# stecrotti/MPSKit.jl

Hardware: AMD Instinct MI355X
Metric: DMRG sweeps/sec + ddAC matvec achieved-TFLOP/s, Heisenberg L=100 D=1024 fp64 (higher is better)
Workload: dtype f64; 1 GPU; Heisenberg S=1/2 FiniteMPS L=100 D=1024 d=2 W=5 fp64, 1-site DMRG sweep (2L-2 site updates), fixed Krylov budget 8 matvecs/site; parallelism=single GPU

## Files before the change

mpskit.jl_amd/csrc/mpsk_api.hip:

```cpp
#include <hip/hip_runtime.h>
#include <cstdio>
#include <cstdlib>
#include <cstring>
#include <cmath>
#include <algorithm>
#include <map>
#include <string>
#include <vector>
#include "mpsk.h"
#include "mpsk_internal.h"

using namespace mpsk;

static thread_local std::string g_err;
static int fail(int code, const std::string& msg) { g_err = msg; return code; }
#define HIPCHK(expr)                                                                        \
  do {                                                                                      \
    hipError_t e_ = (expr);                                                                 \
    if (e_ != hipSuccess)                                                                   \
      return fail(MPSK_ERR_HIP, std::string(#expr) + ": " + hipGetErrorString(e_));         \
  } while (0)
#define REQUIRE(cond, msg)                                                  \
  do {                                                                      \
    if (!(cond)) return fail(MPSK_ERR_INVALID, std::string(__func__) + ": " + (msg)); \
// ... 1074 lines not shown
  for (int q = 0; q < nblk; ++q) { g1.segA[q] = (int64_t)q * kb * Dlo; g1.segB[q] = (int64_t)q * kb * d * Dr; }
  g1.tag = 1;
  HIPCHK(gemm_f64(g1, c->stream));
  GemmArgs g3 = mk(T1, h->GRc, (double*)y, Dlo, Dr, Dr, (int64_t)Dlo * d, Dr, (int64_t)Dlo * d);
  g3.batch = d; g3.bsA = 0; g3.bsB = 0; g3.bsC = (int64_t)Dlo;
  g3.nseg = ns; g3.zsegA = h->zseg; g3.zsegB = h->zseg + (size_t)d * ns;
  g3.tabs_even = (Dlo % 2 == 0) && (Dr % 2 == 0);
  g3.tag = 1;
  HIPCHK(gemm_f64(g3, c->stream));
  return MPSK_OK;
}

int mpsk_hac_eigsolve_fixed(mpsk_hac* h, const void* x0, int m, void* const* V, void* scal, void* y, void* first_image) {
  REQUIRE(h && x0 && V && scal && y, "NULL argument");
  REQUIRE(m >= 1 && m <= 32, "needs 1 <= m <= 32");
  REQUIRE(h->mode != 2, "mpsk_hac_eigsolve_fixed: MPSK_F64 operators only");
  mpsk_ctx* c = h->ctx;
  HIPCHK(hipSetDevice(c->device));
  const int64_t n = (int64_t)h->Dlo * h->H->d * h->Dr;
  REQUIRE(h->Dlo == h->Dl, "mpsk_hac_eigsolve_fixed: the operator must be square (unsharded)");
  double* slot = (double*)scal;
  const int stride = 2 * m + 1;
  double* rbuf = slot + (size_t)m * stride;
  if (int rc = mpsk_vnormalize_dev(c, n, x0, V[0], nullptr)) return rc;
  for (int k = 0; k < m; ++k) {
    if (int rc = mpsk_hac_apply(h, V[k], 1, V[k + 1])) return rc;
    if (k == 0 && first_image) HIPCHK(hipMemcpyAsync(first_image, V[1], sizeof(double) * n, hipMemcpyDeviceToDevice, c->stream));
    HIPCHK(vec_cgs2((const double* const*)V, k + 1, (double*)V[k + 1], n, slot + (size_t)k * stride, c->d_partial, c->stream));
    HIPCHK(vec_scal_rsqrt_dev(slot + (size_t)k * stride + 2 * (k + 1), (double*)V[k + 1], n, c->stream));
  }
  HIPCHK(vec_ritz_small(slot, m, stride, rbuf, rbuf + 32, c->stream));
  HIPCHK(hipMemsetAsync(V[m + 1], 0, sizeof(double) * n, c->stream));
  HIPCHK(vec_multiaxpy((const double* const*)V, rbuf, m, 1.0, (double*)V[m + 1], n, c->stream));
  return mpsk_vnormalize_dev(c, n, V[m + 1], y, nullptr);
}

int mpsk_dC(mpsk_ctx* c, int W, int Dlo, int Dl, int Dr, const void* GL, const void* GR, const void* cm, void* y) {
  REQUIRE(c && GL && GR && cm && y, "NULL argument");
  REQUIRE(W > 0 && Dlo > 0 && Dl > 0 && Dr > 0, "dimensions must be positive");
  if (c->dtype == MPSK_C128)
    return dC_c128(c, W, Dlo, Dl, Dr, (const double*)GL, (const double*)GR, (const double*)cm, (double*)y);
  HIPCHK(hipSetDevice(c->device));
  const size_t slab = (size_t)Dlo * Dr;
  if (int rc = ensure_ws(c, sizeof(double) * slab * W)) return rc;
  double* T1 = (double*)c->ws;
  GemmArgs g1 = mk((const double*)GL, (const double*)cm, T1, Dlo, Dr, Dl, Dlo, Dl, Dlo);
  g1.batch = W; g1.bsA = (int64_t)Dlo * Dl; g1.bsB = 0; g1.bsC = (int64_t)slab;
  g1.tag = 1;
  HIPCHK(gemm_f64(g1, c->stream));
  std::vector<int64_t> sa, sb;
  for (int w = 0; w < W; ++w) { sa.push_back((int64_t)w * slab); sb.push_back((int64_t)w * Dr * Dr); }
  GemmArgs g3 = mk(T1, (const double*)GR, (double*)y, Dlo, Dr, Dr, Dlo, Dr, Dlo);
  g3.tag = 1;
  HIPCHK(gemm_segments(g3, sa, sb, c->stream));
  return MPSK_OK;
}

// ... 1398 lines not shown
  REQUIRE(n > 0, "bad n");
  REQUIRE(((uintptr_t)x % 16 == 0) && ((uintptr_t)y % 16 == 0), "operands must be 16-byte aligned");
  HIPCHK(hipSetDevice(c->device));
  HIPCHK(vec_diff_nrm2((const double*)x, (const double*)y, c->dtype == MPSK_C128 ? 2 * n : n, c->d_scal, c->d_partial,
                       c->stream));
  return fetch_scalars(c, 2, host_out);
}

int mpsk_vgs_step(mpsk_ctx* c, int64_t n, int k, const void* const* xs, void* y, double* host_out) {
  REQUIRE(c && xs && y && host_out, "NULL argument");
  REQUIRE(k > 0 && k <= MAXK && n > 0, "bad k or n");
  HIPCHK(hipSetDevice(c->device));
  HIPCHK(vec_multidot((const double* const*)xs, k, (const double*)y, n, c->d_scal, c->d_partial, c->stream));
  HIPCHK(vec_multiaxpy((const double* const*)xs, c->d_scal, k, -1.0, (double*)y, n, c->stream));
  return fetch_scalars(c, k, host_out);
}

int mpsk_vorth_step(mpsk_ctx* c, int64_t n, int k, const void* const* xs, void* y, double* host_h, double* host_beta) {
  REQUIRE(c && xs && y && host_h && host_beta, "NULL argument");
  REQUIRE(k > 0 && 2 * k + 1 <= MAXK && n > 0, "bad k or n");
  HIPCHK(hipSetDevice(c->device));
  const double* const* X = (const double* const*)xs;
  double* yy = (double*)y;
  HIPCHK(vec_cgs2(X, k, yy, n, c->d_scal, c->d_partial, c->stream));
  HIPCHK(vec_scal_rsqrt_dev(c->d_scal + 2 * k, yy, n, c->stream));
  double tmp[MAXK];
  if (int rc = fetch_scalars(c, 2 * k + 1, tmp)) return rc;
  for (int j = 0; j < k; ++j) host_h[j] = tmp[j] + tmp[k + j];
  *host_beta = tmp[2 * k] > 0.0 ? std::sqrt(tmp[2 * k]) : 0.0;
  return MPSK_OK;
}

int mpsk_vorth_step_dev(mpsk_ctx* c, int64_t n, int k, const void* const* xs, void* y, void* dev_out) {
  REQUIRE(c && xs && y && dev_out, "NULL argument");
  REQUIRE(k > 0 && 2 * k + 1 <= MAXK && n > 0, "bad k or n");
  HIPCHK(hipSetDevice(c->device));
  const double* const* X = (const double* const*)xs;
  double* yy = (double*)y;
  double* out = (double*)dev_out;
  HIPCHK(vec_cgs2(X, k, yy, n, out, c->d_partial, c->stream));
  HIPCHK(vec_scal_rsqrt_dev(out + 2 * k, yy, n, c->stream));
  return MPSK_OK;
}

int mpsk_vlincomb(mpsk_ctx* c, int64_t n, int k, const void* const* xs, const double* host_coefs, void* y) {
  REQUIRE(c && xs && y && host_coefs, "NULL argument");
  REQUIRE(k > 0 && k <= MAXK && n > 0, "bad k or n");
  HIPCHK(hipSetDevice(c->device));
  if (c->coef_pending) { HIPCHK(hipEventSynchronize(c->ev_coef)); c->coef_pending = false; }
  std::memcpy(c->h_coef, host_coefs, sizeof(double) * k);
  HIPCHK(hipMemcpyAsync(c->d_coef, c->h_coef, sizeof(double) * k, hipMemcpyHostToDevice, c->stream));
  HIPCHK(hipEventRecord(c->ev_coef, c->stream));
  c->coef_pending = true;
  HIPCHK(hipMemsetAsync(y, 0, sizeof(double) * n, c->stream));
  HIPCHK(vec_multiaxpy((const double* const*)xs, c->d_coef, k, 1.0, (double*)y, n, c->stream));
  return MPSK_OK;
}

int mpsk_vmultilincomb(mpsk_ctx* c, int64_t n, int k, const void* const* xs, int m, void* const* ys, const double* host_coefs) {
  REQUIRE(c && xs && ys && host_coefs, "NULL argument");
  REQUIRE(k > 0 && k <= 32 && m > 0 && m <= 32 && n > 0, "needs 0 < k, m <= 32 and n > 0");
  for (int j = 0; j < m; ++j)
    for (int i = 0; i < k; ++i) REQUIRE(ys[j] != xs[i], "outputs must not alias inputs");
  HIPCHK(hipSetDevice(c->device));
// ... 8 lines not shown

int mpsk_vritz_dev(mpsk_ctx* c, int m, int stride, const void* dev_slot, void* dev_coef, void* dev_info) {
  REQUIRE(c && dev_slot && dev_coef, "NULL argument");
  REQUIRE(m > 0 && m <= 32 && stride >= 2 * m + 1, "needs 0 < m <= 32 and stride >= 2 m + 1");
  HIPCHK(hipSetDevice(c->device));
  HIPCHK(vec_ritz_small((const double*)dev_slot, m, stride, (double*)dev_coef, (double*)dev_info, c->stream));
  return MPSK_OK;
}

int mpsk_vlincomb_dev(mpsk_ctx* c, int64_t n, int k, const void* const* xs, const void* dev_coefs, void* y) {
  REQUIRE(c && xs && y && dev_coefs, "NULL argument");
  REQUIRE(k > 0 && k <= MAXK && n > 0, "bad k or n");
  HIPCHK(hipSetDevice(c->device));
  HIPCHK(hipMemsetAsync(y, 0, sizeof(double) * n, c->stream));
  HIPCHK(vec_multiaxpy((const double* const*)xs, (const double*)dev_coefs, k, 1.0, (double*)y, n, c->stream));
  return MPSK_OK;
}

int mpsk_vnormalize_dev(mpsk_ctx* c, int64_t n, const void* x, void* y, void* dev_n2) {
  REQUIRE(c && x && y, "NULL argument");
  REQUIRE(n > 0, "bad n");
  HIPCHK(hipSetDevice(c->device));
  double* n2 = dev_n2 ? (double*)dev_n2 : c->d_scal + (MAXK - 1);
  const double* xs[1] = {(const double*)x};
  HIPCHK(vec_multidot(xs, 1, (const double*)x, n, n2, c->d_partial, c->stream));
  if (y != x) HIPCHK(vec_scal_rsqrt_dev_oop(n2, (const double*)x, (double*)y, n, c->stream));
  else HIPCHK(vec_scal_rsqrt_dev(n2, (double*)y, n, c->stream));
  return MPSK_OK;
}

int mpsk_vnrm2_dev(mpsk_ctx* c, int64_t n, const void* x, void* dev_out) {
  REQUIRE(c && x && dev_out, "NULL argument");
  REQUIRE(n > 0, "bad n");
  HIPCHK(hipSetDevice(c->device));
  const double* xs[1] = {(const double*)x};
  HIPCHK(vec_multidot(xs, 1, (const double*)x, n, (double*)dev_out, c->d_partial, c->stream));
  return MPSK_OK;
}

int mpsk_vaxpby(mpsk_ctx* c, int64_t n, double alpha, const void* x, double beta, void* y) {
  REQUIRE(c && x && y, "NULL argument");
  HIPCHK(hipSetDevice(c->device));
  HIPCHK(vec_axpby(alpha, (const double*)x, beta, (double*)y, n, c->stream));
  return MPSK_OK;
}
int mpsk_vscal(mpsk_ctx* c, int64_t n, double alpha, void* x) {
  REQUIRE(c && x, "NULL argument");
  HIPCHK(hipSetDevice(c->device));
  HIPCHK(vec_scal(alpha, (double*)x, n, c->stream));
  return MPSK_OK;
// ... 316 lines not shown
```

mpskit.jl_amd/csrc/mpsk_internal.h:

```cpp
#pragma once
#include <hip/hip_runtime.h>
#include <stdint.h>
#include <stddef.h>
#include <atomic>
#include <vector>
#include <string>

namespace mpsk {

inline hipError_t ensure_dyn_smem(std::atomic<uint64_t>& done, const void* kernel, size_t bytes) {
  int dev = 0;
  hipError_t e = hipGetDevice(&dev);
  if (e != hipSuccess) return e;
  const uint64_t bit = 1ull << (dev & 63);
  if (done.load(std::memory_order_acquire) & bit) return hipSuccess;
  e = hipFuncSetAttribute(kernel, hipFuncAttributeMaxDynamicSharedMemorySize, (int)bytes);
  if (e != hipSuccess) return e;
  done.fetch_or(bit, std::memory_order_release);
  return hipSuccess;
}

constexpr int MAXSEG = 32;

struct GemmArgs {
// ... 43 lines not shown
struct MixTerm { int32_t out, in; double coef; double coef_im = 0.0; };

struct MixPlan {
  int n_out = 0, n_in = 0;
  int32_t* d_rowptr = nullptr;
  int32_t* d_src = nullptr;
  double* d_coef = nullptr;
  double* d_coef_im = nullptr;
  int nnz = 0;
  int max_terms = 0;
};

hipError_t mix_plan_create(const std::vector<MixTerm>& terms, int n_out, int n_in, MixPlan* plan);
void mix_plan_destroy(MixPlan* plan);

struct SlabIndex { int n0, n1; int64_t s0, s1, s2; int64_t ld; };
hipError_t mix_apply(const MixPlan& plan, const double* in, SlabIndex iin, double* out, SlabIndex iout,
                     int R, int C, hipStream_t s);
hipError_t deinterleave(const double* z, int64_t n, double* re, double* im, hipStream_t s);
hipError_t copy_strided(const double* src, int64_t srs, int64_t scs, double* dst, int64_t drs, int64_t dcs, int64_t R,
                        int64_t C, hipStream_t s);
hipError_t identity_slab(double* G, int n, hipStream_t s);

constexpr int MPSK_DOT_SCRATCH = 32 * 1024;
hipError_t vec_multidot(const double* const* xs, int k, const double* y, int64_t n, double* d_out,
                        double* d_partial, hipStream_t s);
hipError_t vec_diff_nrm2(const double* x, const double* y, int64_t n, double* d_out, double* d_partial, hipStream_t s);
hipError_t vec_axpby(double a, const double* x, double b, double* y, int64_t n, hipStream_t s);
hipError_t vec_times_i(const double* x, double* y, int64_t n, hipStream_t s);
hipError_t vec_scal(double a, double* x, int64_t n, hipStream_t s);
hipError_t vec_scal_rsqrt_dev(const double* d_n2, double* x, int64_t n, hipStream_t s);
hipError_t vec_scal_rsqrt_dev_oop(const double* d_n2, const double* x, double* y, int64_t n, hipStream_t s);
hipError_t vec_cgs2(const double* const* xs, int k, double* y, int64_t n, double* d_out, double* d_partial, hipStream_t s);
hipError_t vec_ritz_small(const double* d_slot, int m, int stride, double* d_coef, double* d_info, hipStream_t s);
hipError_t vec_multilincomb(const double* const* xs, int k, double* const* ys, int m, const double* d_coefs, int64_t n,
                            hipStream_t s);
hipError_t vec_multiaxpy(const double* const* xs, const double* d_coefs, int k, double sign, double* y,
                         int64_t n, hipStream_t s);

size_t regularize_workspace_doubles(int W, int D1, int D2);
hipError_t regularize(int W, int D1, int D2, double* v, const double* lvec, const double* rvec, double* partial, hipStream_t s);
hipError_t transpose(const double* in, int ldi, int rows, int cols, double* out, int ldo, hipStream_t s);
size_t qrpos_workspace_doubles(int m, int n);
hipError_t qrpos(int m, int n, const double* A, int lda, double* Q, int ldq, double* R, int ldr, double* ws,
                 hipStream_t s, std::string* err);

size_t cholqr_workspace_doubles(int m, int n);
hipError_t cholqr3(int m, int n, const double* A, int lda, double* Q, int ldq, double* R, int ldr, double* ws,
                   int* d_flag, int* flag_out, hipStream_t s, double shift_scale = 1.0);
hipError_t cholqr_robust(int m, int n, const double* A, int lda, double* Q, int ldq, double* R, int ldr, double* ws,
                         int* d_flag, int* flag_out, hipStream_t s);
hipError_t cholqr1_orth(int m, int n, const double* X, int ldx, double* Q, int ldq, double* ws, int* d_flag, hipStream_t s,
                        double shift_scale);
hipError_t cholqr3_enqueue(int m, int n, const double* A, int lda, double* Q, int ldq, double* R, int ldr, double* ws,
                           int* d_flag, int* flag_out, hipStream_t s, double shift_scale = 1.0);
hipError_t cholqr3_finalize(int m, int n, double* Q, int ldq, double* R, int ldr, double* ws, int* d_flag,
// ... 13 lines not shown
```

mpskit.jl_amd/csrc/mpsk_ops.hip:

```cpp
#include <hip/hip_runtime.h>
#include "mpsk_internal.h"

namespace mpsk {

typedef double d2 __attribute__((ext_vector_type(2)));

__device__ inline int64_t slab_off(const SlabIndex& ix, int j) {
  int j0 = j % ix.n0;
  int t = j / ix.n0;
  int j1 = t % ix.n1;
  int j2 = t / ix.n1;
  return j0 * ix.s0 + j1 * ix.s1 + j2 * ix.s2;
}

template <bool VEC2>
__global__ __launch_bounds__(256) void mix_kernel(const int32_t* __restrict__ rowptr,
                                                  const int32_t* __restrict__ src,
                                                  const double* __restrict__ coef,
                                                  const double* __restrict__ coef_im,
                                                  const double* __restrict__ in, SlabIndex iin,
                                                  double* __restrict__ out, SlabIndex iout, int R, int C) {
  const int o = blockIdx.y;
  const int t0 = rowptr[o], t1 = rowptr[o + 1];
  double* op = out + slab_off(iout, o);
// ... 144 lines not shown
__device__ inline double wave_sum(double v) {
#pragma unroll
  for (int off = 32; off > 0; off >>= 1) v += __shfl_down(v, off, 64);
  return v;
}

template <int NV> __device__ inline void block_sum(double (&v)[NV], double* sh ) {
  const int lane = threadIdx.x & 63, wave = threadIdx.x >> 6;
#pragma unroll
  for (int i = 0; i < NV; ++i) {
    double w = wave_sum(v[i]);
    if (lane == 0) sh[wave * NV + i] = w;
  }
  __syncthreads();
  if (threadIdx.x == 0) {
#pragma unroll
    for (int i = 0; i < NV; ++i) v[i] = sh[i] + sh[NV + i] + sh[2 * NV + i] + sh[3 * NV + i];
  }
  __syncthreads();
}

constexpr int DOT_BLOCKS = 1024;
constexpr int MD = 8;

struct PtrPack { const double* p[MD]; };

template <int NVEC>
__global__ __launch_bounds__(256) void multidot_kernel(PtrPack xs, const double* __restrict__ y, int64_t n,
                                                       double* __restrict__ partial) {
  __shared__ double sh[4 * NVEC];
  double acc[NVEC];
#pragma unroll
  for (int j = 0; j < NVEC; ++j) acc[j] = 0.0;
  const int64_t n2 = n >> 1;
  for (int64_t e = blockIdx.x * (int64_t)blockDim.x + threadIdx.x; e < n2; e += (int64_t)gridDim.x * blockDim.x) {
    d2 yv = *reinterpret_cast<const d2*>(y + 2 * e);
#pragma unroll
    for (int j = 0; j < NVEC; ++j) {
      d2 xv = *reinterpret_cast<const d2*>(xs.p[j] + 2 * e);
      acc[j] += xv.x * yv.x + xv.y * yv.y;
    }
  }
  if ((n & 1) && blockIdx.x == 0 && threadIdx.x == 0) {
#pragma unroll
    for (int j = 0; j < NVEC; ++j) acc[j] += xs.p[j][n - 1] * y[n - 1];
  }
// ... 1 lines not shown
  if (threadIdx.x == 0) {
#pragma unroll
    for (int j = 0; j < NVEC; ++j) partial[(int64_t)j * DOT_BLOCKS + blockIdx.x] = acc[j];
  }
}

__global__ __launch_bounds__(256) void dot_final_kernel(const double* __restrict__ partial, int nblocks,
                                                        double* __restrict__ out) {
  __shared__ double sh[4];
  double acc[1] = {0.0};
  const double* p = partial + (int64_t)blockIdx.x * DOT_BLOCKS;
  for (int i = threadIdx.x; i < nblocks; i += blockDim.x) acc[0] += p[i];
  block_sum<1>(acc, sh);
  if (threadIdx.x == 0) out[blockIdx.x] = acc[0];
}

static int dot_grid(int64_t n) {
  int64_t b = (n / 2 + 255) / 256;
  if (b < 1) b = 1;
  if (b > DOT_BLOCKS) b = DOT_BLOCKS;
  return (int)b;
}

hipError_t vec_multidot(const double* const* xs, int k, const double* y, int64_t n, double* d_out,
                        double* d_partial, hipStream_t s) {
  const int nb = dot_grid(n);
  for (int j0 = 0; j0 < k; j0 += MD) {
    int nv = k - j0 < MD ? k - j0 : MD;
    PtrPack pk;
    for (int j = 0; j < MD; ++j) pk.p[j] = xs[j0 + (j < nv ? j : 0)];
    switch (nv) {
      case 1: hipLaunchKernelGGL(multidot_kernel<1>, dim3(nb), dim3(256), 0, s, pk, y, n, d_partial); break;
      case 2: hipLaunchKernelGGL(multidot_kernel<2>, dim3(nb), dim3(256), 0, s, pk, y, n, d_partial); break;
      case 3: hipLaunchKernelGGL(multidot_kernel<3>, dim3(nb), dim3(256), 0, s, pk, y, n, d_partial); break;
      case 4: hipLaunchKernelGGL(multidot_kernel<4>, dim3(nb), dim3(256), 0, s, pk, y, n, d_partial); break;
      case 5: hipLaunchKernelGGL(multidot_kernel<5>, dim3(nb), dim3(256), 0, s, pk, y, n, d_partial); break;
      case 6: hipLaunchKernelGGL(multidot_kernel<6>, dim3(nb), dim3(256), 0, s, pk, y, n, d_partial); break;
      case 7: hipLaunchKernelGGL(multidot_kernel<7>, dim3(nb), dim3(256), 0, s, pk, y, n, d_partial); break;
      default: hipLaunchKernelGGL(multidot_kernel<8>, dim3(nb), dim3(256), 0, s, pk, y, n, d_partial); break;
    }
    hipLaunchKernelGGL(dot_final_kernel, dim3(nv), dim3(256), 0, s, d_partial, nb, d_out + j0);
  }
  return hipGetLastError();
}

__global__ __launch_bounds__(256) void diff_nrm2_kernel(const double* __restrict__ x, const double* __restrict__ y, int64_t n,
                                                        double* __restrict__ partial) {
  __shared__ double sh[4 * 2];
  double acc[2] = {0.0, 0.0};
  const int64_t n2 = n >> 1;
  for (int64_t e = blockIdx.x * (int64_t)blockDim.x + threadIdx.x; e < n2; e += (int64_t)gridDim.x * blockDim.x) {
    const d2 xv = *reinterpret_cast<const d2*>(x + 2 * e);
    const d2 yv = *reinterpret_cast<const d2*>(y + 2 * e);
    const double d0 = xv.x - yv.x, d1 = xv.y - yv.y;
    acc[0] += d0 * d0 + d1 * d1;
    acc[1] += xv.x * xv.x + xv.y * xv.y;
  }
  if ((n & 1) && blockIdx.x == 0 && threadIdx.x == 0) {
    const double dl = x[n - 1] - y[n - 1];
    acc[0] += dl * dl;
    acc[1] += x[n - 1] * x[n - 1];
  }
  block_sum<2>(acc, sh);
  if (threadIdx.x == 0) {
    partial[blockIdx.x] = acc[0];
    partial[DOT_BLOCKS + blockIdx.x] = acc[1];
  }
}

hipError_t vec_diff_nrm2(const double* x, const double* y, int64_t n, double* d_out, double* d_partial, hipStream_t s) {
  const int nb = dot_grid(n);
  hipLaunchKernelGGL(diff_nrm2_kernel, dim3(nb), dim3(256), 0, s, x, y, n, d_partial);
  hipLaunchKernelGGL(dot_final_kernel, dim3(2), dim3(256), 0, s, d_partial, nb, d_out);
  return hipGetLastError();
}

template <int NVEC, bool NORM>
__global__ __launch_bounds__(256) void multiaxpy_dot_kernel(PtrPack xs, const double* __restrict__ coefs, double sign,
                                                            double* __restrict__ y, int64_t n, double* __restrict__ partial) {
  constexpr int NA = NORM ? 1 : NVEC;
  __shared__ double sh[4 * NA];
  double c[NVEC], acc[NA];
#pragma unroll
  for (int j = 0; j < NVEC; ++j) c[j] = sign * coefs[j];
#pragma unroll
  for (int j = 0; j < NA; ++j) acc[j] = 0.0;
  const int64_t n2 = n >> 1;
  for (int64_t e = blockIdx.x * (int64_t)blockDim.x + threadIdx.x; e < n2; e += (int64_t)gridDim.x * blockDim.x) {
    d2 yv = *reinterpret_cast<const d2*>(y + 2 * e);
    d2 xv[NVEC];
#pragma unroll
    for (int j = 0; j < NVEC; ++j) {
      xv[j] = *reinterpret_cast<const d2*>(xs.p[j] + 2 * e);
      yv.x += c[j] * xv[j].x;
      yv.y += c[j] * xv[j].y;
    }
    *reinterpret_cast<d2*>(y + 2 * e) = yv;
    if (NORM) acc[0] += yv.x * yv.x + yv.y * yv.y;
    else {
#pragma unroll
      for (int j = 0; j < NVEC; ++j) acc[NORM ? 0 : j] += xv[j].x * yv.x + xv[j].y * yv.y;
    }
  }
  if ((n & 1) && blockIdx.x == 0 && threadIdx.x == 0) {
    double v = y[n - 1];
#pragma unroll
    for (int j = 0; j < NVEC; ++j) v += c[j] * xs.p[j][n - 1];
    y[n - 1] = v;
    if (NORM) acc[0] += v * v;
    else {
#pragma unroll
      for (int j = 0; j < NVEC; ++j) acc[NORM ? 0 : j] += xs.p[j][n - 1] * v;
    }
  }
  block_sum<NA>(acc, sh);
  if (threadIdx.x == 0) {
#pragma unroll
    for (int j = 0; j < NA; ++j) partial[(int64_t)j * DOT_BLOCKS + blockIdx.x] = acc[j];
  }
}

template <bool NORM>
static void launch_axpy_dot(int nv, int nb, const PtrPack& pk, const double* cf, double sign, double* y, int64_t n,
                            double* d_partial, hipStream_t s) {
  switch (nv) {
    case 1: hipLaunchKernelGGL((multiaxpy_dot_kernel<1, NORM>), dim3(nb), dim3(256), 0, s, pk, cf, sign, y, n, d_partial); break;
    case 2: hipLaunchKernelGGL((multiaxpy_dot_kernel<2, NORM>), dim3(nb), dim3(256), 0, s, pk, cf, sign, y, n, d_partial); break;
    case 3: hipLaunchKernelGGL((multiaxpy_dot_kernel<3, NORM>), dim3(nb), dim3(256), 0, s, pk, cf, sign, y, n, d_partial); break;
    case 4: hipLaunchKernelGGL((multiaxpy_dot_kernel<4, NORM>), dim3(nb), dim3(256), 0, s, pk, cf, sign, y, n, d_partial); break;
    case 5: hipLaunchKernelGGL((multiaxpy_dot_kernel<5, NORM>), dim3(nb), dim3(256), 0, s, pk, cf, sign, y, n, d_partial); break;
    case 6: hipLaunchKernelGGL((multiaxpy_dot_kernel<6, NORM>), dim3(nb), dim3(256), 0, s, pk, cf, sign, y, n, d_partial); break;
    case 7: hipLaunchKernelGGL((multiaxpy_dot_kernel<7, NORM>), dim3(nb), dim3(256), 0, s, pk, cf, sign, y, n, d_partial); break;
    default: hipLaunchKernelGGL((multiaxpy_dot_kernel<8, NORM>), dim3(nb), dim3(256), 0, s, pk, cf, sign, y, n, d_partial); break;
  }
}

constexpr int ML = 32;
struct PtrPackL { const double* p[ML]; };

template <int NVEC>
__global__ __launch_bounds__(256) void multiaxpy_dot_long_kernel(PtrPackL xs, const double* __restrict__ coefs, double sign,
                                                                 double* __restrict__ y, int64_t n, int k,
                                                                 double* __restrict__ partial) {
  __shared__ double sh[4 * NVEC];
  double c[NVEC], acc[NVEC];
#pragma unroll
  for (int j = 0; j < NVEC; ++j) { c[j] = j < k ? sign * coefs[j] : 0.0; acc[j] = 0.0; }
  for (int64_t e = blockIdx.x * (int64_t)blockDim.x + threadIdx.x; e < n; e += (int64_t)gridDim.x * blockDim.x) {
    double yv = y[e];
    double xv[NVEC];
#pragma unroll
    for (int j = 0; j < NVEC; ++j) {
      xv[j] = xs.p[j][e];
      yv += c[j] * xv[j];
    }
    y[e] = yv;
#pragma unroll
    for (int j = 0; j < NVEC; ++j) acc[j] += xv[j] * yv;
  }
  block_sum<NVEC>(acc, sh);
  if (threadIdx.x == 0) {
#pragma unroll
    for (int j = 0; j < NVEC; ++j)
      if (j < k) partial[(int64_t)j * DOT_BLOCKS + blockIdx.x] = acc[j];
  }
}

__global__ __launch_bounds__(256) void multiaxpy_norm_long_kernel(PtrPackL xs, const double* __restrict__ coefs, double sign,
                                                                  double* __restrict__ y, int64_t n, int k,
                                                                  double* __restrict__ partial) {
  __shared__ double sh[4];
  __shared__ double cs[ML];
  if (threadIdx.x < ML) cs[threadIdx.x] = threadIdx.x < k ? sign * coefs[threadIdx.x] : 0.0;
  __syncthreads();
  double acc[1] = {0.0};
  for (int64_t e = blockIdx.x * (int64_t)blockDim.x + threadIdx.x; e < n; e += (int64_t)gridDim.x * blockDim.x) {
    double yv = y[e];
    for (int j = 0; j < k; ++j) yv += cs[j] * xs.p[j][e];
    y[e] = yv;
    acc[0] += yv * yv;
  }
  block_sum<1>(acc, sh);
  if (threadIdx.x == 0) partial[blockIdx.x] = acc[0];
}

static int dot_grid_long(int64_t n) {
  int64_t b = (n + 255) / 256;
  if (b < 1) b = 1;
  if (b > DOT_BLOCKS) b = DOT_BLOCKS;
  return (int)b;
}

hipError_t vec_cgs2(const double* const* xs, int k, double* y, int64_t n, double* d_out, double* d_partial, hipStream_t s) {
  if (n <= 0 || k <= 0) return hipErrorInvalidValue;
  hipError_t e = vec_multidot(xs, k, y, n, d_out, d_partial, s);
  if (e != hipSuccess) return e;
  if (k > MD && k <= ML) {
    const int nbl = dot_grid_long(n);
    PtrPackL pk;
    for (int j = 0; j < ML; ++j) pk.p[j] = xs[j < k ? j : 0];
    if (k <= 16) hipLaunchKernelGGL(multiaxpy_dot_long_kernel<16>, dim3(nbl), dim3(256), 0, s, pk, d_out, -1.0, y, n, k, d_partial);
    else if (k <= 24) hipLaunchKernelGGL(multiaxpy_dot_long_kernel<24>, dim3(nbl), dim3(256), 0, s, pk, d_out, -1.0, y, n, k, d_partial);
    else hipLaunchKernelGGL(multiaxpy_dot_long_kernel<32>, dim3(nbl), dim3(256), 0, s, pk, d_out, -1.0, y, n, k, d_partial);
    hipLaunchKernelGGL(dot_final_kernel, dim3(k), dim3(256), 0, s, d_partial, nbl, d_out + k);
    hipLaunchKernelGGL(multiaxpy_norm_long_kernel, dim3(nbl), dim3(256), 0, s, pk, d_out + k, -1.0, y, n, k, d_partial);
    hipLaunchKernelGGL(dot_final_kernel, dim3(1), dim3(256), 0, s, d_partial, nbl, d_out + 2 * k);
    return hipGetLastError();
  }
  if (k > MD) {
    if ((e = vec_multiaxpy(xs, d_out, k, -1.0, y, n, s)) != hipSuccess) return e;
    if ((e = vec_multidot(xs, k, y, n, d_out + k, d_partial, s)) != hipSuccess) return e;
    if ((e = vec_multiaxpy(xs, d_out + k, k, -1.0, y, n, s)) != hipSuccess) return e;
    const double* ys[1] = {y};
    return vec_multidot(ys, 1, y, n, d_out + 2 * k, d_partial, s);
  }
  const int nb = dot_grid(n);
  PtrPack pk;
  for (int j = 0; j < MD; ++j) pk.p[j] = xs[j < k ? j : 0];
  launch_axpy_dot<false>(k, nb, pk, d_out, -1.0, y, n, d_partial, s);
  hipLaunchKernelGGL(dot_final_kernel, dim3(k), dim3(256), 0, s, d_partial, nb, d_out + k);
  launch_axpy_dot<true>(k, nb, pk, d_out + k, -1.0, y, n, d_partial, s);
  hipLaunchKernelGGL(dot_final_kernel, dim3(1), dim3(256), 0, s, d_partial, nb, d_out + 2 * k);
  return hipGetLastError();
}

__global__ __launch_bounds__(256) void axpby_kernel(double a, const double* __restrict__ x, double b,
                                                    double* __restrict__ y, int64_t n) {
  const int64_t n2 = n >> 1;
  for (int64_t e = blockIdx.x * (int64_t)blockDim.x + threadIdx.x; e < n2; e += (int64_t)gridDim.x * blockDim.x) {
    d2 xv = *reinterpret_cast<const d2*>(x + 2 * e);
    d2 r;
    if (b == 0.0) { r.x = a * xv.x; r.y = a * xv.y; }
    else {
      d2 yv = *reinterpret_cast<const d2*>(y + 2 * e);
      r.x = a * xv.x + b * yv.x; r.y = a * xv.y + b * yv.y;
    }
    *reinterpret_cast<d2*>(y + 2 * e) = r;
  }
  if ((n & 1) && blockIdx.x == 0 && threadIdx.x == 0)
    y[n - 1] = (b == 0.0) ? a * x[n - 1] : a * x[n - 1] + b * y[n - 1];
}

__global__ __launch_bounds__(256) void times_i_kernel(const double* __restrict__ x, double* __restrict__ y, int64_t npairs) {
  typedef double d2 __attribute__((ext_vector_type(2)));
  for (int64_t e = blockIdx.x * (int64_t)blockDim.x + threadIdx.x; e < npairs; e += (int64_t)gridDim.x * blockDim.x) {
    const d2 v = reinterpret_cast<const d2*>(x)[e];
    reinterpret_cast<d2*>(y)[e] = d2{-v.y, v.x};
  }
}
hipError_t vec_times_i(const double* x, double* y, int64_t n, hipStream_t s) {
  const int64_t npairs = n / 2;
  int64_t nb = (npairs + 255) / 256;
  if (nb > 4096) nb = 4096;
  if (nb < 1) nb = 1;
  hipLaunchKernelGGL(times_i_kernel, dim3((int)nb), dim3(256), 0, s, x, y, npairs);
  return hipGetLastError();
}

__global__ __launch_bounds__(256) void scal_kernel(double a, double* x, int64_t n) {
  for (int64_t e = blockIdx.x * (int64_t)blockDim.x + threadIdx.x; e < n; e += (int64_t)gridDim.x * blockDim.x)
    x[e] *= a;
}

__global__ __launch_bounds__(256) void scal_rsqrt_dev_kernel(const double* __restrict__ d_n2, double* x, int64_t n) {
  const double n2 = *d_n2;
  const double a = (n2 > 0.0) ? 1.0 / sqrt(n2) : 0.0;
  for (int64_t e = blockIdx.x * (int64_t)blockDim.x + threadIdx.x; e < n; e += (int64_t)gridDim.x * blockDim.x)
    x[e] *= a;
}

__global__ __launch_bounds__(256) void scal_rsqrt_dev_oop_kernel(const double* __restrict__ d_n2, const double* __restrict__ x,
                                                                 double* __restrict__ y, int64_t n) {
  const double n2 = *d_n2;
  const double a = (n2 > 0.0) ? 1.0 / sqrt(n2) : 0.0;
  for (int64_t e = blockIdx.x * (int64_t)blockDim.x + threadIdx.x; e < n; e += (int64_t)gridDim.x * blockDim.x)
    y[e] = a * x[e];
}
hipError_t vec_scal_rsqrt_dev_oop(const double* d_n2, const double* x, double* y, int64_t n, hipStream_t s) {
  if (n <= 0) return hipSuccess;
  int64_t nb = (n + 255) / 256;
  if (nb > 4096) nb = 4096;
  hipLaunchKernelGGL(scal_rsqrt_dev_oop_kernel, dim3((int)nb), dim3(256), 0, s, d_n2, x, y, n);
  return hipGetLastError();
}

hipError_t vec_scal_rsqrt_dev(const double* d_n2, double* x, int64_t n, hipStream_t s) {
  if (n <= 0) return hipSuccess;
  int64_t nb = (n + 255) / 256;
  if (nb > 4096) nb = 4096;
  hipLaunchKernelGGL(scal_rsqrt_dev_kernel, dim3((int)nb), dim3(256), 0, s, d_n2, x, n);
  return hipGetLastError();
}

constexpr int RITZ_MAX = 32;
__device__ __forceinline__ double ritz_rcp(double x) {
  double r = __builtin_amdgcn_rcp(x);
  r = r * (2.0 - x * r);
  return r * (2.0 - x * r);
}
__device__ __forceinline__ double ritz_rsq(double x) {
  double r = __builtin_amdgcn_rsq(x);
  r = r * (1.5 - 0.5 * x * r * r);
  return r * (1.5 - 0.5 * x * r * r);
}
__global__ __launch_bounds__(64) void ritz_small_kernel(const double* __restrict__ slot, int m, int stride,
                                                        double* __restrict__ coef, double* __restrict__ info) {
  __shared__ double A[RITZ_MAX][RITZ_MAX + 1], V[RITZ_MAX][RITZ_MAX + 1], beta[RITZ_MAX];
  __shared__ int meff_s, rp[RITZ_MAX / 2], rq[RITZ_MAX / 2];
  __shared__ double rc[RITZ_MAX / 2], rs[RITZ_MAX / 2];
  const int t = threadIdx.x;
  for (int e = t; e < RITZ_MAX * RITZ_MAX; e += 64) { A[e / RITZ_MAX][e % RITZ_MAX] = 0.0; V[e / RITZ_MAX][e % RITZ_MAX] = (e / RITZ_MAX == e % RITZ_MAX) ? 1.0 : 0.0; }
  __syncthreads();
  if (t < m) {
// ... 194 lines not shown
```

Before: 1.146 sweeps/s.

## Fold dot-product final reductions into consumer kernels and fuse Krylov copy/lincomb steps

Removes the separate dot_final reduction kernels by having each consuming kernel (axpy-dot, norm, rsqrt scaling) re-reduce the per-block partials at its start. It double-buffers the partial scratch, writes the first matvec image directly and reads it as a CGS source so the device-to-device copy disappears, and fuses the final Ritz linear combination with zero-init and normalization. This cuts kernel launches and serialization on the latency-bound small-vector Krylov path, at the cost of every block redundantly summing up to 1024 partials per coefficient.

```diff
diff --git a/mpskit.jl_amd/csrc/mpsk_api.hip b/mpskit.jl_amd/csrc/mpsk_api.hip
--- a/mpskit.jl_amd/csrc/mpsk_api.hip
+++ b/mpskit.jl_amd/csrc/mpsk_api.hip
@@ -1120,17 +1120,17 @@
   double* slot = (double*)scal;
   const int stride = 2 * m + 1;
   double* rbuf = slot + (size_t)m * stride;
-  if (int rc = mpsk_vnormalize_dev(c, n, x0, V[0], nullptr)) return rc;
+  double* n2 = c->d_scal + (MAXK - 1);
+  HIPCHK(vec_normalize_dev((const double*)x0, (double*)V[0], n, n2, c->d_partial, c->stream));
   for (int k = 0; k < m; ++k) {
-    if (int rc = mpsk_hac_apply(h, V[k], 1, V[k + 1])) return rc;
-    if (k == 0 && first_image) HIPCHK(hipMemcpyAsync(first_image, V[1], sizeof(double) * n, hipMemcpyDeviceToDevice, c->stream));
-    HIPCHK(vec_cgs2((const double* const*)V, k + 1, (double*)V[k + 1], n, slot + (size_t)k * stride, c->d_partial, c->stream));
-    HIPCHK(vec_scal_rsqrt_dev(slot + (size_t)k * stride + 2 * (k + 1), (double*)V[k + 1], n, c->stream));
+    double* img = (k == 0 && first_image) ? (double*)first_image : (double*)V[k + 1];
+    if (int rc = mpsk_hac_apply(h, V[k], 1, img)) return rc;
+    HIPCHK(vec_cgs2_normalize((const double* const*)V, k + 1, img, (double*)V[k + 1], n, slot + (size_t)k * stride, c->d_partial,
+                              c->stream));
   }
   HIPCHK(vec_ritz_small(slot, m, stride, rbuf, rbuf + 32, c->stream));
-  HIPCHK(hipMemsetAsync(V[m + 1], 0, sizeof(double) * n, c->stream));
-  HIPCHK(vec_multiaxpy((const double* const*)V, rbuf, m, 1.0, (double*)V[m + 1], n, c->stream));
-  return mpsk_vnormalize_dev(c, n, V[m + 1], y, nullptr);
+  HIPCHK(vec_lincomb_normalize((const double* const*)V, rbuf, m, (double*)V[m + 1], (double*)y, n, n2, c->d_partial, c->stream));
+  return MPSK_OK;
 }
 
 int mpsk_dC(mpsk_ctx* c, int W, int Dlo, int Dl, int Dr, const void* GL, const void* GR, const void* cm, void* y) {
@@ -2575,8 +2575,7 @@
   HIPCHK(hipSetDevice(c->device));
   const double* const* X = (const double* const*)xs;
   double* yy = (double*)y;
-  HIPCHK(vec_cgs2(X, k, yy, n, c->d_scal, c->d_partial, c->stream));
-  HIPCHK(vec_scal_rsqrt_dev(c->d_scal + 2 * k, yy, n, c->stream));
+  HIPCHK(vec_cgs2_normalize(X, k, yy, yy, n, c->d_scal, c->d_partial, c->stream));
   double tmp[MAXK];
   if (int rc = fetch_scalars(c, 2 * k + 1, tmp)) return rc;
   for (int j = 0; j < k; ++j) host_h[j] = tmp[j] + tmp[k + j];
@@ -2591,8 +2590,7 @@
   const double* const* X = (const double* const*)xs;
   double* yy = (double*)y;
   double* out = (double*)dev_out;
-  HIPCHK(vec_cgs2(X, k, yy, n, out, c->d_partial, c->stream));
-  HIPCHK(vec_scal_rsqrt_dev(out + 2 * k, yy, n, c->stream));
+  HIPCHK(vec_cgs2_normalize(X, k, yy, yy, n, out, c->d_partial, c->stream));
   return MPSK_OK;
 }
 
@@ -2647,10 +2645,7 @@
   REQUIRE(n > 0, "bad n");
   HIPCHK(hipSetDevice(c->device));
   double* n2 = dev_n2 ? (double*)dev_n2 : c->d_scal + (MAXK - 1);
-  const double* xs[1] = {(const double*)x};
-  HIPCHK(vec_multidot(xs, 1, (const double*)x, n, n2, c->d_partial, c->stream));
-  if (y != x) HIPCHK(vec_scal_rsqrt_dev_oop(n2, (const double*)x, (double*)y, n, c->stream));
-  else HIPCHK(vec_scal_rsqrt_dev(n2, (double*)y, n, c->stream));
+  HIPCHK(vec_normalize_dev((const double*)x, (double*)y, n, n2, c->d_partial, c->stream));
   return MPSK_OK;
 }
 
diff --git a/mpskit.jl_amd/csrc/mpsk_internal.h b/mpskit.jl_amd/csrc/mpsk_internal.h
--- a/mpskit.jl_amd/csrc/mpsk_internal.h
+++ b/mpskit.jl_amd/csrc/mpsk_internal.h
@@ -89,7 +89,8 @@
                         int64_t C, hipStream_t s);
 hipError_t identity_slab(double* G, int n, hipStream_t s);
 
-constexpr int MPSK_DOT_SCRATCH = 32 * 1024;
+constexpr int MPSK_DOT_HALF = 32 * 1024;
+constexpr int MPSK_DOT_SCRATCH = 2 * MPSK_DOT_HALF;
 hipError_t vec_multidot(const double* const* xs, int k, const double* y, int64_t n, double* d_out,
                         double* d_partial, hipStream_t s);
 hipError_t vec_diff_nrm2(const double* x, const double* y, int64_t n, double* d_out, double* d_partial, hipStream_t s);
@@ -97,8 +98,12 @@
 hipError_t vec_times_i(const double* x, double* y, int64_t n, hipStream_t s);
 hipError_t vec_scal(double a, double* x, int64_t n, hipStream_t s);
 hipError_t vec_scal_rsqrt_dev(const double* d_n2, double* x, int64_t n, hipStream_t s);
-hipError_t vec_scal_rsqrt_dev_oop(const double* d_n2, const double* x, double* y, int64_t n, hipStream_t s);
-hipError_t vec_cgs2(const double* const* xs, int k, double* y, int64_t n, double* d_out, double* d_partial, hipStream_t s);
+hipError_t vec_multidot_partials(const double* const* xs, int k, const double* y, int64_t n, double* partial, hipStream_t s);
+hipError_t vec_cgs2_normalize(const double* const* xs, int k, const double* ysrc, double* y, int64_t n, double* d_out,
+                              double* d_partial, hipStream_t s);
+hipError_t vec_lincomb_normalize(const double* const* xs, const double* d_coefs, int k, double* y, double* out, int64_t n,
+                                 double* d_n2, double* d_partial, hipStream_t s);
+hipError_t vec_normalize_dev(const double* x, double* y, int64_t n, double* d_n2, double* d_partial, hipStream_t s);
 hipError_t vec_ritz_small(const double* d_slot, int m, int stride, double* d_coef, double* d_info, hipStream_t s);
 hipError_t vec_multilincomb(const double* const* xs, int k, double* const* ys, int m, const double* d_coefs, int64_t n,
                             hipStream_t s);
diff --git a/mpskit.jl_amd/csrc/mpsk_ops.hip b/mpskit.jl_amd/csrc/mpsk_ops.hip
--- a/mpskit.jl_amd/csrc/mpsk_ops.hip
+++ b/mpskit.jl_amd/csrc/mpsk_ops.hip
@@ -190,6 +190,8 @@
 
 constexpr int DOT_BLOCKS = 1024;
 constexpr int MD = 8;
+constexpr int ML_ROWS = 32;
+static_assert(ML_ROWS * DOT_BLOCKS == MPSK_DOT_HALF, "partial-buffer half must hold ML rows of DOT_BLOCKS sums");
 
 struct PtrPack { const double* p[MD]; };
 
@@ -237,6 +239,38 @@
   return (int)b;
 }
 
+template <int NV>
+__device__ inline void finish_partials(const double* __restrict__ pin, int nblocks, int nv, double* sh ,
+                                       double* bc ) {
+  double v[NV];
+#pragma unroll
+  for (int j = 0; j < NV; ++j) v[j] = 0.0;
+  for (int i = threadIdx.x; i < nblocks; i += 256) {
+#pragma unroll
+    for (int j = 0; j < NV; ++j)
+      if (j < nv) v[j] += pin[(int64_t)j * DOT_BLOCKS + i];
+  }
+  block_sum<NV>(v, sh);
+  if (threadIdx.x == 0) {
+#pragma unroll
+    for (int j = 0; j < NV; ++j) bc[j] = v[j];
+  }
+  __syncthreads();
+}
+
+static void launch_multidot(int nv, int nb, const PtrPack& pk, const double* y, int64_t n, double* partial, hipStream_t s) {
+  switch (nv) {
+    case 1: hipLaunchKernelGGL(multidot_kernel<1>, dim3(nb), dim3(256), 0, s, pk, y, n, partial); break;
+    case 2: hipLaunchKernelGGL(multidot_kernel<2>, dim3(nb), dim3(256), 0, s, pk, y, n, partial); break;
+    case 3: hipLaunchKernelGGL(multidot_kernel<3>, dim3(nb), dim3(256), 0, s, pk, y, n, partial); break;
+    case 4: hipLaunchKernelGGL(multidot_kernel<4>, dim3(nb), dim3(256), 0, s, pk, y, n, partial); break;
+    case 5: hipLaunchKernelGGL(multidot_kernel<5>, dim3(nb), dim3(256), 0, s, pk, y, n, partial); break;
+    case 6: hipLaunchKernelGGL(multidot_kernel<6>, dim3(nb), dim3(256), 0, s, pk, y, n, partial); break;
+    case 7: hipLaunchKernelGGL(multidot_kernel<7>, dim3(nb), dim3(256), 0, s, pk, y, n, partial); break;
+    default: hipLaunchKernelGGL(multidot_kernel<8>, dim3(nb), dim3(256), 0, s, pk, y, n, partial); break;
+  }
+}
+
 hipError_t vec_multidot(const double* const* xs, int k, const double* y, int64_t n, double* d_out,
                         double* d_partial, hipStream_t s) {
   const int nb = dot_grid(n);
@@ -244,17 +278,20 @@
     int nv = k - j0 < MD ? k - j0 : MD;
     PtrPack pk;
     for (int j = 0; j < MD; ++j) pk.p[j] = xs[j0 + (j < nv ? j : 0)];
-    switch (nv) {
-      case 1: hipLaunchKernelGGL(multidot_kernel<1>, dim3(nb), dim3(256), 0, s, pk, y, n, d_partial); break;
-      case 2: hipLaunchKernelGGL(multidot_kernel<2>, dim3(nb), dim3(256), 0, s, pk, y, n, d_partial); break;
-      case 3: hipLaunchKernelGGL(multidot_kernel<3>, dim3(nb), dim3(256), 0, s, pk, y, n, d_partial); break;
-      case 4: hipLaunchKernelGGL(multidot_kernel<4>, dim3(nb), dim3(256), 0, s, pk, y, n, d_partial); break;
-      case 5: hipLaunchKernelGGL(multidot_kernel<5>, dim3(nb), dim3(256), 0, s, pk, y, n, d_partial); break;
-      case 6: hipLaunchKernelGGL(multidot_kernel<6>, dim3(nb), dim3(256), 0, s, pk, y, n, d_partial); break;
-      case 7: hipLaunchKernelGGL(multidot_kernel<7>, dim3(nb), dim3(256), 0, s, pk, y, n, d_partial); break;
-      default: hipLaunchKernelGGL(multidot_kernel<8>, dim3(nb), dim3(256), 0, s, pk, y, n, d_partial); break;
-    }
+    launch_multidot(nv, nb, pk, y, n, d_partial, s);
     hipLaunchKernelGGL(dot_final_kernel, dim3(nv), dim3(256), 0, s, d_partial, nb, d_out + j0);
+  }
+  return hipGetLastError();
+}
+
+hipError_t vec_multidot_partials(const double* const* xs, int k, const double* y, int64_t n, double* partial, hipStream_t s) {
+  if (k <= 0 || k > ML_ROWS) return hipErrorInvalidValue;
+  const int nb = dot_grid(n);
+  for (int j0 = 0; j0 < k; j0 += MD) {
+    int nv = k - j0 < MD ? k - j0 : MD;
+    PtrPack pk;
+    for (int j = 0; j < MD; ++j) pk.p[j] = xs[j0 + (j < nv ? j : 0)];
+    launch_multidot(nv, nb, pk, y, n, partial + (int64_t)j0 * DOT_BLOCKS, s);
   }
   return hipGetLastError();
 }
@@ -291,18 +328,31 @@
 }
 
 template <int NVEC, bool NORM>
-__global__ __launch_bounds__(256) void multiaxpy_dot_kernel(PtrPack xs, const double* __restrict__ coefs, double sign,
-                                                            double* __restrict__ y, int64_t n, double* __restrict__ partial) {
+__global__ __launch_bounds__(256) void multiaxpy_dot_kernel(PtrPack xs, double* d_cf, const double* __restrict__ pin,
+                                                            int pin_nb, double sign, const double* ysrc, double* y,
+                                                            int64_t n, double* __restrict__ partial) {
   constexpr int NA = NORM ? 1 : NVEC;
-  __shared__ double sh[4 * NA];
+  __shared__ double sh[4 * NVEC];
+  __shared__ double bc[NVEC];
   double c[NVEC], acc[NA];
-#pragma unroll
-  for (int j = 0; j < NVEC; ++j) c[j] = sign * coefs[j];
+  if (pin) {
+    finish_partials<NVEC>(pin, pin_nb, NVEC, sh, bc);
+#pragma unroll
+    for (int j = 0; j < NVEC; ++j) {
+      const double cf = bc[j];
+      if (blockIdx.x == 0 && threadIdx.x == 0) d_cf[j] = cf;
+      c[j] = sign * cf;
+    }
+  } else {
+#pragma unroll
+    for (int j = 0; j < NVEC; ++j) c[j] = sign * d_cf[j];
+  }
 #pragma unroll
   for (int j = 0; j < NA; ++j) acc[j] = 0.0;
   const int64_t n2 = n >> 1;
   for (int64_t e = blockIdx.x * (int64_t)blockDim.x + threadIdx.x; e < n2; e += (int64_t)gridDim.x * blockDim.x) {
-    d2 yv = *reinterpret_cast<const d2*>(y + 2 * e);
+    d2 yv = {0.0, 0.0};
+    if (ysrc) yv = *reinterpret_cast<const d2*>(ysrc + 2 * e);
     d2 xv[NVEC];
 #pragma unroll
     for (int j = 0; j < NVEC; ++j) {
@@ -318,7 +368,7 @@
     }
   }
   if ((n & 1) && blockIdx.x == 0 && threadIdx.x == 0) {
-    double v = y[n - 1];
+    double v = ysrc ? ysrc[n - 1] : 0.0;
 #pragma unroll
     for (int j = 0; j < NVEC; ++j) v += c[j] * xs.p[j][n - 1];
     y[n - 1] = v;
@@ -336,31 +386,42 @@
 }
 
 template <bool NORM>
-static void launch_axpy_dot(int nv, int nb, const PtrPack& pk, const double* cf, double sign, double* y, int64_t n,
-                            double* d_partial, hipStream_t s) {
+static void launch_axpy_dot(int nv, int nb, const PtrPack& pk, double* cf, const double* pin, int pin_nb, double sign,
+                            const double* ysrc, double* y, int64_t n, double* d_partial, hipStream_t s) {
+#define MPSK_AXPY_DOT(NV) \
+  hipLaunchKernelGGL((multiaxpy_dot_kernel<NV, NORM>), dim3(nb), dim3(256), 0, s, pk, cf, pin, pin_nb, sign, ysrc, y, n, d_partial)
   switch (nv) {
-    case 1: hipLaunchKernelGGL((multiaxpy_dot_kernel<1, NORM>), dim3(nb), dim3(256), 0, s, pk, cf, sign, y, n, d_partial); break;
-    case 2: hipLaunchKernelGGL((multiaxpy_dot_kernel<2, NORM>), dim3(nb), dim3(256), 0, s, pk, cf, sign, y, n, d_partial); break;
-    case 3: hipLaunchKernelGGL((multiaxpy_dot_kernel<3, NORM>), dim3(nb), dim3(256), 0, s, pk, cf, sign, y, n, d_partial); break;
-    case 4: hipLaunchKernelGGL((multiaxpy_dot_kernel<4, NORM>), dim3(nb), dim3(256), 0, s, pk, cf, sign, y, n, d_partial); break;
-    case 5: hipLaunchKernelGGL((multiaxpy_dot_kernel<5, NORM>), dim3(nb), dim3(256), 0, s, pk, cf, sign, y, n, d_partial); break;
-    case 6: hipLaunchKernelGGL((multiaxpy_dot_kernel<6, NORM>), dim3(nb), dim3(256), 0, s, pk, cf, sign, y, n, d_partial); break;
-    case 7: hipLaunchKernelGGL((multiaxpy_dot_kernel<7, NORM>), dim3(nb), dim3(256), 0, s, pk, cf, sign, y, n, d_partial); break;
-    default: hipLaunchKernelGGL((multiaxpy_dot_kernel<8, NORM>), dim3(nb), dim3(256), 0, s, pk, cf, sign, y, n, d_partial); break;
-  }
+    case 1: MPSK_AXPY_DOT(1); break;
+    case 2: MPSK_AXPY_DOT(2); break;
+    case 3: MPSK_AXPY_DOT(3); break;
+    case 4: MPSK_AXPY_DOT(4); break;
+    case 5: MPSK_AXPY_DOT(5); break;
+    case 6: MPSK_AXPY_DOT(6); break;
+    case 7: MPSK_AXPY_DOT(7); break;
+    default: MPSK_AXPY_DOT(8); break;
+  }
+#undef MPSK_AXPY_DOT
 }
 
 constexpr int ML = 32;
+static_assert(ML == ML_ROWS, "partial-buffer rows");
 struct PtrPackL { const double* p[ML]; };
 
 template <int NVEC>
-__global__ __launch_bounds__(256) void multiaxpy_dot_long_kernel(PtrPackL xs, const double* __restrict__ coefs, double sign,
-                                                                 double* __restrict__ y, int64_t n, int k,
-                                                                 double* __restrict__ partial) {
+__global__ __launch_bounds__(256) void multiaxpy_dot_long_kernel(PtrPackL xs, double* d_cf, const double* __restrict__ pin,
+                                                                 int pin_nb, double sign, double* __restrict__ y, int64_t n,
+                                                                 int k, double* __restrict__ partial) {
   __shared__ double sh[4 * NVEC];
+  __shared__ double bc[NVEC];
   double c[NVEC], acc[NVEC];
-#pragma unroll
-  for (int j = 0; j < NVEC; ++j) { c[j] = j < k ? sign * coefs[j] : 0.0; acc[j] = 0.0; }
+  finish_partials<NVEC>(pin, pin_nb, k, sh, bc);
+#pragma unroll
+  for (int j = 0; j < NVEC; ++j) {
+    const double cf = bc[j];
+    if (j < k && blockIdx.x == 0 && threadIdx.x == 0) d_cf[j] = cf;
+    c[j] = j < k ? sign * cf : 0.0;
+    acc[j] = 0.0;
+  }
   for (int64_t e = blockIdx.x * (int64_t)blockDim.x + threadIdx.x; e < n; e += (int64_t)gridDim.x * blockDim.x) {
     double yv = y[e];
     double xv[NVEC];
@@ -381,12 +442,19 @@
   }
 }
 
-__global__ __launch_bounds__(256) void multiaxpy_norm_long_kernel(PtrPackL xs, const double* __restrict__ coefs, double sign,
-                                                                  double* __restrict__ y, int64_t n, int k,
-                                                                  double* __restrict__ partial) {
-  __shared__ double sh[4];
+__global__ __launch_bounds__(256) void multiaxpy_norm_long_kernel(PtrPackL xs, double* d_cf, const double* __restrict__ pin,
+                                                                  int pin_nb, double sign, double* __restrict__ y, int64_t n,
+                                                                  int k, double* __restrict__ partial) {
+  __shared__ double sh[4 * MD];
+  __shared__ double bc[ML];
   __shared__ double cs[ML];
-  if (threadIdx.x < ML) cs[threadIdx.x] = threadIdx.x < k ? sign * coefs[threadIdx.x] : 0.0;
+  for (int j0 = 0; j0 < k; j0 += MD)
+    finish_partials<MD>(pin + (int64_t)j0 * DOT_BLOCKS, pin_nb, k - j0 < MD ? k - j0 : MD, sh, bc + j0);
+  if (threadIdx.x < ML) {
+    const double cf = bc[threadIdx.x];
+    if ((int)threadIdx.x < k && blockIdx.x == 0) d_cf[threadIdx.x] = cf;
+    cs[threadIdx.x] = (int)threadIdx.x < k ? sign * cf : 0.0;
+  }
   __syncthreads();
   double acc[1] = {0.0};
   for (int64_t e = blockIdx.x * (int64_t)blockDim.x + threadIdx.x; e < n; e += (int64_t)gridDim.x * blockDim.x) {
@@ -406,37 +474,63 @@
   return (int)b;
 }
 
-hipError_t vec_cgs2(const double* const* xs, int k, double* y, int64_t n, double* d_out, double* d_partial, hipStream_t s) {
+static hipError_t scal_rsqrt_partials(const double* pin, int pin_nb, double* d_n2, const double* x, double* y, int64_t n,
+                                      hipStream_t s);
+
+hipError_t vec_cgs2_normalize(const double* const* xs, int k, const double* ysrc, double* y, int64_t n, double* d_out,
+                              double* d_partial, hipStream_t s) {
   if (n <= 0 || k <= 0) return hipErrorInvalidValue;
-  hipError_t e = vec_multidot(xs, k, y, n, d_out, d_partial, s);
-  if (e != hipSuccess) return e;
-  if (k > MD && k <= ML) {
-    const int nbl = dot_grid_long(n);
-    PtrPackL pk;
-    for (int j = 0; j < ML; ++j) pk.p[j] = xs[j < k ? j : 0];
-    if (k <= 16) hipLaunchKernelGGL(multiaxpy_dot_long_kernel<16>, dim3(nbl), dim3(256), 0, s, pk, d_out, -1.0, y, n, k, d_partial);
-    else if (k <= 24) hipLaunchKernelGGL(multiaxpy_dot_long_kernel<24>, dim3(nbl), dim3(256), 0, s, pk, d_out, -1.0, y, n, k, d_partial);
-    else hipLaunchKernelGGL(multiaxpy_dot_long_kernel<32>, dim3(nbl), dim3(256), 0, s, pk, d_out, -1.0, y, n, k, d_partial);
-    hipLaunchKernelGGL(dot_final_kernel, dim3(k), dim3(256), 0, s, d_partial, nbl, d_out + k);
-    hipLaunchKernelGGL(multiaxpy_norm_long_kernel, dim3(nbl), dim3(256), 0, s, pk, d_out + k, -1.0, y, n, k, d_partial);
-    hipLaunchKernelGGL(dot_final_kernel, dim3(1), dim3(256), 0, s, d_partial, nbl, d_out + 2 * k);
-    return hipGetLastError();
-  }
-  if (k > MD) {
+  if (ysrc != y && k > MD) return hipErrorInvalidValue;
+  hipError_t e;
+  if (k > ML) {
+    if ((e = vec_multidot(xs, k, y, n, d_out, d_partial, s)) != hipSuccess) return e;
     if ((e = vec_multiaxpy(xs, d_out, k, -1.0, y, n, s)) != hipSuccess) return e;
     if ((e = vec_multidot(xs, k, y, n, d_out + k, d_partial, s)) != hipSuccess) return e;
     if ((e = vec_multiaxpy(xs, d_out + k, k, -1.0, y, n, s)) != hipSuccess) return e;
     const double* ys[1] = {y};
-    return vec_multidot(ys, 1, y, n, d_out + 2 * k, d_partial, s);
-  }
+    if ((e = vec_multidot(ys, 1, y, n, d_out + 2 * k, d_partial, s)) != hipSuccess) return e;
+    return vec_scal_rsqrt_dev(d_out + 2 * k, y, n, s);
+  }
+  double* const p0 = d_partial;
+  double* const p1 = d_partial + MPSK_DOT_HALF;
   const int nb = dot_grid(n);
+  if ((e = vec_multidot_partials(xs, k, ysrc, n, p0, s)) != hipSuccess) return e;
+  if (k > MD) {
+    const int nbl = dot_grid_long(n);
+    PtrPackL pk;
+    for (int j = 0; j < ML; ++j) pk.p[j] = xs[j < k ? j : 0];
+    if (k <= 16) hipLaunchKernelGGL(multiaxpy_dot_long_kernel<16>, dim3(nbl), dim3(256), 0, s, pk, d_out, p0, nb, -1.0, y, n, k, p1);
+    else if (k <= 24) hipLaunchKernelGGL(multiaxpy_dot_long_kernel<24>, dim3(nbl), dim3(256), 0, s, pk, d_out, p0, nb, -1.0, y, n, k, p1);
+    else hipLaunchKernelGGL(multiaxpy_dot_long_kernel<32>, dim3(nbl), dim3(256), 0, s, pk, d_out, p0, nb, -1.0, y, n, k, p1);
+    hipLaunchKernelGGL(multiaxpy_norm_long_kernel, dim3(nbl), dim3(256), 0, s, pk, d_out + k, p1, nbl, -1.0, y, n, k, p0);
+    return scal_rsqrt_partials(p0, nbl, d_out + 2 * k, y, y, n, s);
+  }
   PtrPack pk;
   for (int j = 0; j < MD; ++j) pk.p[j] = xs[j < k ? j : 0];
-  launch_axpy_dot<false>(k, nb, pk, d_out, -1.0, y, n, d_partial, s);
-  hipLaunchKernelGGL(dot_final_kernel, dim3(k), dim3(256), 0, s, d_partial, nb, d_out + k);
-  launch_axpy_dot<true>(k, nb, pk, d_out + k, -1.0, y, n, d_partial, s);
-  hipLaunchKernelGGL(dot_final_kernel, dim3(1), dim3(256), 0, s, d_partial, nb, d_out + 2 * k);
-  return hipGetLastError();
+  launch_axpy_dot<false>(k, nb, pk, d_out, p0, nb, -1.0, ysrc, y, n, p1, s);
+  launch_axpy_dot<true>(k, nb, pk, d_out + k, p1, nb, -1.0, y, y, n, p0, s);
+  return scal_rsqrt_partials(p0, nb, d_out + 2 * k, y, y, n, s);
+}
+
+hipError_t vec_lincomb_normalize(const double* const* xs, const double* d_coefs, int k, double* y, double* out, int64_t n,
+                                 double* d_n2, double* d_partial, hipStream_t s) {
+  if (n <= 0 || k <= 0) return hipErrorInvalidValue;
+  const int nb = dot_grid(n);
+  for (int j0 = 0; j0 < k; j0 += MD) {
+    int nv = k - j0 < MD ? k - j0 : MD;
+    PtrPack pk;
+    for (int j = 0; j < MD; ++j) pk.p[j] = xs[j0 + (j < nv ? j : 0)];
+    launch_axpy_dot<true>(nv, nb, pk, const_cast<double*>(d_coefs) + j0, nullptr, 0, 1.0, j0 ? y : nullptr, y, n, d_partial, s);
+  }
+  return scal_rsqrt_partials(d_partial, nb, d_n2, y, out, n, s);
+}
+
+hipError_t vec_normalize_dev(const double* x, double* y, int64_t n, double* d_n2, double* d_partial, hipStream_t s) {
+  if (n <= 0) return hipErrorInvalidValue;
+  const double* xs[1] = {x};
+  hipError_t e = vec_multidot_partials(xs, 1, x, n, d_partial, s);
+  if (e != hipSuccess) return e;
+  return scal_rsqrt_partials(d_partial, dot_grid(n), d_n2, x, y, n, s);
 }
 
 __global__ __launch_bounds__(256) void axpby_kernel(double a, const double* __restrict__ x, double b,
@@ -477,33 +571,47 @@
     x[e] *= a;
 }
 
-__global__ __launch_bounds__(256) void scal_rsqrt_dev_kernel(const double* __restrict__ d_n2, double* x, int64_t n) {
-  const double n2 = *d_n2;
+__global__ __launch_bounds__(256) void scal_rsqrt_dev_kernel(double* d_n2, const double* __restrict__ pin, int pin_nb, double* x,
+                                                             int64_t n) {
+  __shared__ double sh[4];
+  __shared__ double bc[1];
+  double n2;
+  if (pin) {
+    finish_partials<1>(pin, pin_nb, 1, sh, bc);
+    n2 = bc[0];
+    if (blockIdx.x == 0 && threadIdx.x == 0) *d_n2 = n2;
+  } else n2 = *d_n2;
   const double a = (n2 > 0.0) ? 1.0 / sqrt(n2) : 0.0;
   for (int64_t e = blockIdx.x * (int64_t)blockDim.x + threadIdx.x; e < n; e += (int64_t)gridDim.x * blockDim.x)
     x[e] *= a;
 }
 
-__global__ __launch_bounds__(256) void scal_rsqrt_dev_oop_kernel(const double* __restrict__ d_n2, const double* __restrict__ x,
-                                                                 double* __restrict__ y, int64_t n) {
-  const double n2 = *d_n2;
+__global__ __launch_bounds__(256) void scal_rsqrt_dev_oop_kernel(double* d_n2, const double* __restrict__ pin, int pin_nb,
+                                                                 const double* __restrict__ x, double* __restrict__ y, int64_t n) {
+  __shared__ double sh[4];
+  __shared__ double bc[1];
+  finish_partials<1>(pin, pin_nb, 1, sh, bc);
+  const double n2 = bc[0];
+  if (blockIdx.x == 0 && threadIdx.x == 0) *d_n2 = n2;
   const double a = (n2 > 0.0) ? 1.0 / sqrt(n2) : 0.0;
   for (int64_t e = blockIdx.x * (int64_t)blockDim.x + threadIdx.x; e < n; e += (int64_t)gridDim.x * blockDim.x)
     y[e] = a * x[e];
 }
-hipError_t vec_scal_rsqrt_dev_oop(const double* d_n2, const double* x, double* y, int64_t n, hipStream_t s) {
-  if (n <= 0) return hipSuccess;
+static int scal_grid(int64_t n) {
   int64_t nb = (n + 255) / 256;
   if (nb > 4096) nb = 4096;
-  hipLaunchKernelGGL(scal_rsqrt_dev_oop_kernel, dim3((int)nb), dim3(256), 0, s, d_n2, x, y, n);
-  return hipGetLastError();
-}
-
+  return (int)nb;
+}
 hipError_t vec_scal_rsqrt_dev(const double* d_n2, double* x, int64_t n, hipStream_t s) {
   if (n <= 0) return hipSuccess;
-  int64_t nb = (n + 255) / 256;
-  if (nb > 4096) nb = 4096;
-  hipLaunchKernelGGL(scal_rsqrt_dev_kernel, dim3((int)nb), dim3(256), 0, s, d_n2, x, n);
+  hipLaunchKernelGGL(scal_rsqrt_dev_kernel, dim3(scal_grid(n)), dim3(256), 0, s, const_cast<double*>(d_n2), nullptr, 0, x, n);
+  return hipGetLastError();
+}
+
+static hipError_t scal_rsqrt_partials(const double* pin, int pin_nb, double* d_n2, const double* x, double* y, int64_t n,
+                                      hipStream_t s) {
+  if (y == x) hipLaunchKernelGGL(scal_rsqrt_dev_kernel, dim3(scal_grid(n)), dim3(256), 0, s, d_n2, pin, pin_nb, y, n);
+  else hipLaunchKernelGGL(scal_rsqrt_dev_oop_kernel, dim3(scal_grid(n)), dim3(256), 0, s, d_n2, pin, pin_nb, x, y, n);
   return hipGetLastError();
 }
 
```

Result: no change. 1.152 sweeps/s (median of 6 runs) (+0.5%).
